# ShujiaHuang/basevar

Measured on AMD Instinct MI355X. Metric: genomic sites/sec through basetype caller at N samples, higher is better.
Workload: dtype f64

## Files before the change

basevar_amd/_capi.py:

```python
import ctypes as C
import os

import numpy as np

HERE = os.path.dirname(os.path.abspath(__file__))
LIB_PATH = os.environ.get("BASEVAR_AMD_LIB") or os.path.join(HERE, "lib", "libbasevar_amd.so")

BV_MAX_ALT = 4
BV_MAX_GROUPS = 255
BV_NO_GROUP = 0xFF
BV_MEM_DEVICE, BV_MEM_HOST = 0, 1
BV_SLAB_RPR_TAGGED, BV_RPR_TAG_MAX_RANK = 0x1, 0x1FFF
BV_FLAG_LANES = 0x10000000
BV_FLAG_SPARSE_TIMING = 0x20000000
BV_FORM_SHORT_ROWS, BV_FORM_ONE_KERNEL, BV_FORM_PASS2_FUSED = 0x1, 0x2, 0x4
BV_FLAG_TALLY_ONLY, BV_FLAG_SKIP_FISHER, BV_FLAG_SKIP_LRT, BV_FLAG_TILE_STATE, BV_FLAG_WAVE_SOLVER = 0x1, 0x2, 0x4, 0x8, 0x10
BV_OK, BV_ERR_INVALID_ARG, BV_ERR_NO_DEVICE, BV_ERR_HIP, BV_ERR_TOO_LARGE, BV_ERR_SITE = 0, -1, -2, -3, -4, -5

BV_SITE_COVERED, BV_SITE_VARIANT, BV_SITE_BAD_QUAL = 0x1, 0x2, 0x4
BV_SITE_ZERO_FREQ, BV_SITE_RANKSUM, BV_SITE_SOR_OVERFLOW, BV_SITE_RPR_RANGE = 0x8, 0x10, 0x20, 0x40

BV_CELL_REV, BV_CELL_NOCALL, BV_CELL_N, BV_CELL_INS, BV_CELL_DEL = 0x04, 0x08, 0x08, 0x09, 0x0A

SITE_DTYPE = np.dtype([
    ("depth", "<u4", 4), ("total_depth", "<u4"), ("status", "<u4"),
    ("cvg_sb", "<u4", 4), ("cvg_fs", "<f8"), ("cvg_sor", "<f8"),
    ("n_alt", "u1"), ("alt", "u1", 4), ("n_em", "u1"), ("em_iters", "<u2"),
    ("af", "<f8", 4), ("caf", "<f8", 4), ("qual", "<f8"), ("chi2", "<f8"), ("qd", "<f8"),
    ("var_sb", "<u4", 4), ("var_fs", "<f8"), ("var_sor", "<f8"),
    ("mq_ranksum", "<f8"), ("rpr_ranksum", "<f8"), ("bq_ranksum", "<f8"),
])
GROUP_DTYPE = np.dtype([("n_alt", "u1"), ("alt", "u1", 4), ("reserved", "u1", 3), ("total_depth", "<u4"),
                        ("reserved2", "<u4"), ("af", "<f8", 4)])
assert SITE_DTYPE.itemsize == 208 and GROUP_DTYPE.itemsize == 48


class Slab(C.Structure):
    _fields_ = [("n_sites", C.c_uint32), ("n_samples", C.c_uint32), ("pitch", C.c_uint64),
                ("base_strand", C.c_void_p), ("qual", C.c_void_p), ("mapq", C.c_void_p), ("rpr", C.c_void_p),
                ("ref_base", C.c_void_p), ("group_id", C.c_void_p), ("n_groups", C.c_uint32),
                ("mem_kind", C.c_uint32), ("layout", C.c_uint32), ("reserved_", C.c_uint32)]


class SparseTile(C.Structure):
    _fields_ = [("n_sites", C.c_uint32), ("n_samples", C.c_uint32), ("n_entries", C.c_uint32), ("n_groups", C.c_uint32),
                ("row_start", C.c_void_p), ("sample", C.c_void_p), ("base_strand", C.c_void_p), ("qual", C.c_void_p), ("mapq", C.c_void_p),
                ("rpr", C.c_void_p), ("group_id", C.c_void_p), ("mem_kind", C.c_uint32), ("layout", C.c_uint32)]


class TextRows(C.Structure):
    _fields_ = [("text", C.c_void_p), ("row_off", C.c_void_p), ("file_samples", C.c_void_p), ("text_bytes", C.c_uint64),
                ("n_positions", C.c_uint32), ("n_files", C.c_uint32), ("reserved_", C.c_uint32)]


BV_TEXT_SKIP, BV_TEXT_HOST, BV_TEXT_INDEL = 1, 2, 4


class BgzfMembers(C.Structure):
    _fields_ = [("data", C.c_void_p), ("member_off", C.c_void_p), ("data_bytes", C.c_uint64), ("n_members", C.c_uint32),
                ("reserved_", C.c_uint32)]


class BgzfRows(C.Structure):
    _fields_ = [("data", C.c_void_p), ("member_off", C.c_void_p), ("data_bytes", C.c_uint64), ("file_member", C.c_void_p),
                ("file_samples", C.c_void_p), ("skip_bytes", C.c_void_p), ("skip_lines", C.c_void_p), ("n_files", C.c_uint32),
                ("max_positions", C.c_uint32), ("at_end", C.c_uint32), ("reserved_", C.c_uint32)]

# ... 128 lines not shown
```

basevar_amd/csrc/bv_engine.hip:

```cpp
#include <hip/hip_runtime.h>
#include <link.h>
#include <sched.h>

#include <algorithm>
#include <cctype>
#include <cmath>
#include <cstdio>
#include <cstdlib>
#include <cstring>
#include <mutex>
#include <string>
#include <vector>

#include "bv_engine_impl.h"

void bv_launch_synth(const bv_synth_params &p, uint32_t n_sites, uint32_t n_samples, uint64_t pitch, uint8_t *bs,
                     uint8_t *q, uint8_t *mapq, uint16_t *rpr, uint8_t *ref_base, hipStream_t stream);

namespace {
std::mutex g_err_mu;
std::string g_err;

void set_global_error(const std::string &m) {
    std::lock_guard<std::mutex> lk(g_err_mu);
// ... 351 lines not shown
            e->err = std::string(#call) + ": " + hipGetErrorString(_s);                               \
            return bail(BV_ERR_HIP);                                                                  \
        }                                                                                             \
    } while (0)
    BV_TRY(hipSetDevice(cfg->device));
    e->n_cu = prop.multiProcessorCount > 0 ? (uint32_t)prop.multiProcessorCount : 256u;
    BV_TRY(hipStreamCreateWithFlags(&e->stream, hipStreamNonBlocking));
    BV_TRY(hipEventCreateWithFlags(&e->ev_done, hipEventDisableTiming));
    for (auto &tri : e->ring)
        for (auto &ev : tri) BV_TRY(hipEventCreate(&ev));
    BV_TRY(hipMalloc(&e->d_tables, sizeof(BvTables)));
    BV_TRY(hipMalloc(&e->d_var_list, sizeof(uint32_t) * (size_t)cfg->max_sites));
    BV_TRY(hipMalloc(&e->d_counters, sizeof(uint32_t) * BV_CTR_WORDS * bv_engine::kCtrBlocks));
    BV_TRY(hipHostMalloc(&e->h_counters, sizeof(uint32_t) * BV_CTR_WORDS * bv_engine::kCtrBlocks));
    std::memset(e->h_counters, 0, sizeof(uint32_t) * BV_CTR_WORDS * bv_engine::kCtrBlocks);
    BV_TRY(hipMemset(e->d_counters, 0, sizeof(uint32_t) * BV_CTR_WORDS * bv_engine::kCtrBlocks));

    BvTables t;
    const double MLN10TO10 = -0.23025850929940458;
    for (int qv = 0; qv < BV_QBINS; ++qv) {
        double epsilon = exp((double)qv * MLN10TO10);
        t.hit[qv] = 1.0 - epsilon;
        t.miss[qv] = epsilon / 3;
        t.loghit[qv] = log(t.hit[qv]);
        t.logmiss[qv] = log(t.miss[qv]);
    }
    e->host_log_exact = load_host_log_table(t.hostlog) ? 1 : 0;
    if (!e->host_log_exact) {
        static const char *note =
            "basevar_amd: note: the host libm's log() could not be reproduced on the device (no glibc __log_data table found, or it "
            "failed verification); sites of <= 64 covered samples use the device library's log(): values within 1e-6, exact ties "
            "between allele subsets undecided (records carry BV_SITE_LOG_APPROX)";
        static std::once_flag said;
        std::call_once(said, [] { if (!std::getenv("BASEVAR_AMD_QUIET")) std::fprintf(stderr, "%s\n", note); });
        set_global_error(note);
    }
    {
        size_t nfact = (size_t)(cfg->max_samples ? cfg->max_samples : 1u << 20) + 2;
        if (nfact < (1u << 16)) nfact = 1u << 16;
        if (nfact > (1u << 23)) nfact = 1u << 23;
        std::vector<double> lf(nfact);
        for (size_t k = 0; k < nfact; ++k) {
            int sign;
            lf[k] = lgamma_r((double)k + 1.0, &sign);
        }
        BV_TRY(hipMalloc(&e->d_lnfact, sizeof(double) * nfact));
        BV_TRY(hipMemcpy(e->d_lnfact, lf.data(), sizeof(double) * nfact, hipMemcpyHostToDevice));
        t.lnfact = e->d_lnfact;
        t.lnfact_n = (uint32_t)nfact;
        t.pad_ = 0;
    }
    BV_TRY(hipMemcpy(e->d_tables, &t, sizeof(t), hipMemcpyHostToDevice));
#undef BV_TRY
    if (cfg->flags & BV_FLAG_LANES) {
        if (const char *nl = std::getenv("BASEVAR_AMD_LANES")) e->n_lanes = std::max(2, std::min((int)bv_engine::kMaxLanes, std::atoi(nl)));
        for (int k = 0; k < e->n_lanes; ++k) {
            bv_engine_config c = *cfg;
            c.flags &= ~BV_FLAG_LANES;
            const int rc = bv_engine_create(&c, &e->lane[k]);
            if (rc != BV_OK) {
                const std::string m = bv_last_error(nullptr);
                bv_engine_destroy(e);
                set_global_error("bv_engine_create: lane engine: " + m);
                return rc;
            }
            e->lane[k]->is_lane = true;
        }
    }
    *out = e;
    return BV_OK;
}

int bv_engine_destroy(bv_engine *e) {
    if (!e) return BV_OK;
    (void)hipSetDevice(e->cfg.device);
    for (bv_engine *&l : e->lane) {
        if (l) (void)bv_engine_destroy(l);
        l = nullptr;
    }
    if (e->ev_entry) (void)hipEventDestroy(e->ev_entry);
    if (e->stream) (void)hipStreamSynchronize(e->stream);
    bv_text_state_free(e->text);
    bv_bgzf_state_free(e->bgzf);
    bv_deflate_state_free(e->deflate);
    for (hipStream_t st : e->used_streams) (void)hipStreamSynchronize(st);
    for (auto &tri : e->ring)
        for (auto &ev : tri)
            if (ev) (void)hipEventDestroy(ev);
    if (e->d_tables) (void)hipFree(e->d_tables);
    if (e->d_lnfact) (void)hipFree(e->d_lnfact);
    if (e->d_var_list) (void)hipFree(e->d_var_list);
    if (e->d_counters) (void)hipFree(e->d_counters);
    if (e->d_gid) (void)hipFree(e->d_gid);
    if (e->d_summ) (void)hipFree(e->d_summ);
    if (e->d_bins) (void)hipFree(e->d_bins);
    if (e->d_cand_list) (void)hipFree(e->d_cand_list);
    if (e->d_easy_list) (void)hipFree(e->d_easy_list);
    if (e->d_easy3_list) (void)hipFree(e->d_easy3_list);
    if (e->d_ovf) (void)hipFree(e->d_ovf);
    if (e->d_gitems) (void)hipFree(e->d_gitems);
    if (e->d_gidp) (void)hipFree(e->d_gidp);
    if (e->d_chain) (void)hipFree(e->d_chain);
    if (e->d_ref_cat) (void)hipFree(e->d_ref_cat);
    if (e->d_out_cat) (void)hipFree(e->d_out_cat);
    if (e->ev_done) (void)hipEventDestroy(e->ev_done);
    if (e->ev_host) (void)hipEventDestroy(e->ev_host);
    if (e->h_counters) (void)hipHostFree(e->h_counters);
    for (auto &sl : e->sring) {
        if (sl.buf) (void)hipFree(sl.buf);
        if (sl.copied) (void)hipEventDestroy(sl.copied);
        if (sl.freed) (void)hipEventDestroy(sl.freed);
    }
    tile_job_free(e->tile);
    if (e->d_gid_round) (void)hipFree(e->d_gid_round);
    if (e->d_gout_round) (void)hipFree(e->d_gout_round);
    for (hipStream_t cs : e->copy_stream)
        if (cs) (void)hipStreamSynchronize(cs);
    for (hipStream_t cs : e->copy_stream)
        if (cs) (void)hipStreamDestroy(cs);
    if (e->stream) (void)hipStreamDestroy(e->stream);
    delete e;
    return BV_OK;
}

}

int bv_impl::launch_passes(bv_engine *e, const uint8_t *bs, const uint8_t *q, const uint8_t *mq, const uint16_t *rp, const uint8_t *refb,
                           const uint8_t *gid, size_t P, uint32_t n_sites, uint32_t n_samples, uint32_t n_groups, bv_site_result *dout,
                           bv_group_result *dgout, hipStream_t st, const BvChain *chain, bool chain_cat, uint32_t layout) {
    const uint32_t rpr_tag = (layout & BV_SLAB_RPR_TAGGED) && rp != nullptr ? 1u : 0u;
    const size_t S = n_sites, G = n_groups;
    const size_t Gr = G < BV_GROUPS_PER_ROUND ? G : (size_t)BV_GROUPS_PER_ROUND, n_rounds = G ? (G + Gr - 1) / Gr : 1;
    if (n_rounds > 1 && chain != nullptr) return fail(e, BV_ERR_INVALID_ARG, "launch_passes: more than 32 pop-groups do not chain");
    if (G && chain == nullptr) BV_HIP(e, hipMemsetAsync(dgout, 0, S * G * sizeof(bv_group_result), st));
    if (n_rounds > 1) {
        int rc = grow_device(e, &e->d_gid_round, &e->d_gid_round_bytes, up256(n_samples) + 256);
        if (rc == BV_OK) rc = grow_device(e, &e->d_gout_round, &e->d_gout_round_bytes, S * Gr * sizeof(bv_group_result));
        if (rc != BV_OK) return rc;
    }

    const bool timed = !(e->cfg.flags & BV_FLAG_SPARSE_TIMING) || (e->n_launches % 8u) == 0u;
    e->n_launches += 1;
    hipEvent_t *ev = nullptr;
    if (timed) {
        if (e->ring_count == bv_engine::kRing) {
            int rc = drain_timings(e, true);
            if (rc != BV_OK) return rc;
        }
        const int slot = e->ring_head;
        e->ring_head = (e->ring_head + 1) % bv_engine::kRing;
        e->ring_count += 1;
        e->last_slot = slot;
        ev = e->ring[slot];
        e->ring_one_kernel[slot] = false;
    }
    const bool two_kernel = n_samples <= BV_SHORT_ROW_MAX;

    BvPass2Args a2;
    a2.bs = bs; a2.q = q; a2.mapq = mq; a2.rpr = rp; a2.ref_base = refb; a2.group_id = gid; a2.pitch = P;
    a2.n_sites = n_sites; a2.n_samples = n_samples; a2.n_groups = n_groups;
    a2.min_af = e->cfg.min_af; a2.tables = e->d_tables; a2.out = dout; a2.gout = dgout;
    a2.var_list = e->d_var_list; a2.counters = e->d_counters; a2.n_cu = e->n_cu; a2.flags = e->cfg.flags;
    a2.gitems = nullptr; a2.gitem_cap = 0; a2.gidp = nullptr;
    a2.ch = chain;
    a2.ch_cat = chain_cat ? 1u : 0u;
    a2.rpr_tag = rpr_tag;
    if (G && gid && dgout && !(e->cfg.flags & BV_FLAG_GROUP_INLINE)) {
        const uint64_t want64 = (uint64_t)S * Gr, most = (8192ull << 20) / (sizeof(uint32_t) * BV_P2G_ITEM_WORDS);
        uint32_t want = (uint32_t)(want64 < most ? want64 : most);
        if (want > e->gitem_cap) {
            if (e->d_gitems) BV_HIP(e, hipFree(e->d_gitems));
            e->d_gitems = nullptr; e->gitem_cap = 0;
            for (;;) {
                if (hipMalloc(&e->d_gitems, sizeof(uint32_t) * BV_P2G_ITEM_WORDS * (size_t)want) == hipSuccess) {
                    e->gitem_cap = want;
                    break;
                }
                (void)hipGetLastError();
                e->d_gitems = nullptr;
                if (want < 1024u) break;
                want /= 2u;
            }
        }
        a2.gitems = e->d_gitems; a2.gitem_cap = e->gitem_cap;
        const size_t n16 = ((size_t)n_samples + 15) & ~(size_t)15;
        const int rc = grow_device(e, &e->d_gidp, &e->d_gidp_bytes, n16 + 256);
        if (rc != BV_OK) return rc;
        a2.gidp = e->d_gidp;
        if (n_rounds == 1) {
            bv_launch_gid_prepare(gid, e->d_gidp, (uint32_t)n16, n_groups, st);
            BV_HIP(e, hipGetLastError());
        }
    }
    if (n_rounds > 1) a2.n_groups = (uint32_t)Gr;

    e->last_blocks = 1;
#ifdef BV_TEAM_DEBUG
    const bool rotate = false;
#else
    const bool rotate = true;
#endif
    uint32_t cb = 0;
    if (rotate) {
        cb = e->ctr_rot % bv_engine::kCtrBlocks;
        if (cb == 0)
            BV_HIP(e, hipMemset2DAsync(e->d_counters, sizeof(uint32_t) * BV_CTR_WORDS, 0, sizeof(uint32_t) * BV_CTR_PER_LAUNCH * BV_CTR_STRIDE,
                                       bv_engine::kCtrBlocks, st));
        e->ctr_rot += 1;
    } else {
        e->ctr_rot = 0;
        BV_HIP(e, hipMemsetAsync(e->d_counters, 0, sizeof(uint32_t) * BV_CTR_PER_LAUNCH * BV_CTR_STRIDE, st));
    }
    e->last_ctr_base = cb;
    a2.counters = e->d_counters + (size_t)cb * BV_CTR_WORDS;
    bool pass2_fused = false;
    e->last_form = two_kernel ? BV_FORM_SHORT_ROWS : 0u;
    if (ev) BV_HIP(e, hipEventRecord(ev[0], st));
    if (two_kernel) {
        if (n_sites > e->short_sites) {
            if (e->d_summ) BV_HIP(e, hipFree(e->d_summ));
            if (e->d_bins) BV_HIP(e, hipFree(e->d_bins));
            if (e->d_cand_list) BV_HIP(e, hipFree(e->d_cand_list));
            if (e->d_easy_list) BV_HIP(e, hipFree(e->d_easy_list));
            if (e->d_easy3_list) BV_HIP(e, hipFree(e->d_easy3_list));
            if (e->d_ovf) BV_HIP(e, hipFree(e->d_ovf));
            e->d_ovf = nullptr;
            e->d_summ = nullptr; e->d_bins = nullptr; e->d_cand_list = nullptr; e->d_easy_list = nullptr; e->d_easy3_list = nullptr; e->short_sites = 0;
            BV_HIP(e, hipMalloc(&e->d_summ, sizeof(BvSiteSummary) * (size_t)n_sites));
            BV_HIP(e, hipMalloc(&e->d_bins, sizeof(uint32_t) * BV_S_BIN_STRIDE * (size_t)n_sites));
            BV_HIP(e, hipMalloc(&e->d_cand_list, sizeof(uint32_t) * (size_t)n_sites));
            BV_HIP(e, hipMalloc(&e->d_easy_list, sizeof(uint32_t) * (size_t)n_sites));
            BV_HIP(e, hipMalloc(&e->d_easy3_list, sizeof(uint32_t) * (size_t)n_sites));
            BV_HIP(e, hipMalloc(&e->d_ovf, sizeof(uint32_t) * 4 * (size_t)n_sites));
            e->short_sites = n_sites;
        }
        BvP1ShortArgs s1;
        s1.bs = bs; s1.q = q; s1.ref_base = refb; s1.pitch = P; s1.n_sites = n_sites; s1.n_samples = n_samples;
        s1.flags = e->cfg.flags; s1.n_cu = e->n_cu; s1.min_af = e->cfg.min_af; s1.tables = e->d_tables; s1.out = dout;
        s1.var_list = e->d_var_list; s1.counters = e->d_counters + (size_t)cb * BV_CTR_WORDS;
        s1.summ = e->d_summ; s1.bins = e->d_bins;
        s1.cand_list = e->d_cand_list; s1.easy_list = e->d_easy_list; s1.easy3_list = e->d_easy3_list;
        s1.ovf = e->d_ovf;
        s1.ch = chain;
        s1.mapq = nullptr; s1.rpr = nullptr; s1.rpr_tag = rpr_tag;
        const uint32_t form = (e->cfg.flags >> 12) & 0xFu;
        if (form != 9u && bv_p1s_fused_takes(s1)) {
            if (ev) e->ring_one_kernel[e->last_slot] = true;
            if (form != 10u && mq != nullptr && rp != nullptr && !(e->cfg.flags & BV_FLAG_PASS2_SWEEP)) {
                s1.mapq = mq; s1.rpr = rp;
                pass2_fused = true;
            }
            bv_launch_p1s_fused(s1, st);
            BV_HIP(e, hipGetLastError());
            e->last_form |= BV_FORM_ONE_KERNEL | (pass2_fused ? BV_FORM_PASS2_FUSED : 0u);
        } else {
            bv_launch_p1s_stream(s1, st);
            BV_HIP(e, hipGetLastError());
            if (ev) BV_HIP(e, hipEventRecord(ev[3], st));
            bv_launch_p1s_solve(s1, st);
            BV_HIP(e, hipGetLastError());
        }
        if (ev) BV_HIP(e, hipEventRecord(ev[1], st));
    } else {
        if (ev) e->ring_one_kernel[e->last_slot] = true;
        BvPass1Args a1;
        a1.bs = bs; a1.q = q; a1.ref_base = refb; a1.pitch = P; a1.n_sites = n_sites;
        a1.n_samples = n_samples; a1.flags = e->cfg.flags; a1.min_af = e->cfg.min_af; a1.tables = e->d_tables; a1.out = dout;
        a1.var_list = e->d_var_list; a1.counters = e->d_counters + (size_t)cb * BV_CTR_WORDS; a1.n_cu = e->n_cu;
        a1.ch = chain;
        bv_launch_pass1(a1, st);
        BV_HIP(e, hipGetLastError());
        e->last_form |= BV_FORM_ONE_KERNEL;
        if (ev) BV_HIP(e, hipEventRecord(ev[1], st));
    }

    for (size_t r = 0; r < n_rounds; ++r) {
        const size_t g_lo = r * Gr, g_n = n_rounds > 1 ? std::min(Gr, G - g_lo) : G;
        if (n_rounds > 1) {
            const size_t n16 = ((size_t)n_samples + 15) & ~(size_t)15;
            bv_launch_gid_round(gid, e->d_gid_round, (uint32_t)n16, (uint32_t)g_lo, (uint32_t)g_n, st);
            BV_HIP(e, hipGetLastError());
            bv_launch_gid_prepare(e->d_gid_round, e->d_gidp, (uint32_t)n16, (uint32_t)g_n, st);
            BV_HIP(e, hipGetLastError());
            BV_HIP(e, hipMemsetAsync(e->d_gout_round, 0, S * g_n * sizeof(bv_group_result), st));
        }
        BvPass2Args ac = a2;
        if (n_rounds > 1) { ac.group_id = e->d_gid_round; ac.n_groups = (uint32_t)g_n; ac.gout = e->d_gout_round; }
        if (pass2_fused || r > 0) {
            if (G == 0) continue;
            ac.mapq = nullptr; ac.rpr = nullptr;
        }
        bv_launch_pass2(ac, st);
        BV_HIP(e, hipGetLastError());
        bv_launch_p2g_solve16(ac, st);
        BV_HIP(e, hipGetLastError());
        if (n_rounds > 1)
            BV_HIP(e, hipMemcpy2DAsync(dgout + g_lo, G * sizeof(bv_group_result), e->d_gout_round, g_n * sizeof(bv_group_result),
                                       g_n * sizeof(bv_group_result), S, hipMemcpyDeviceToDevice, st));
    }
    if (ev) BV_HIP(e, hipEventRecord(ev[2], st));

    if (rotate) e->ctr_mirror_stale = true;
    else BV_HIP(e, hipMemcpyAsync(e->h_counters, e->d_counters, sizeof(uint32_t) * BV_CTR_WORDS * bv_engine::kCtrBlocks, hipMemcpyDeviceToHost, st));
    const int rc = copy_records_back(e, st);
    if (rc != BV_OK) return rc;
    e->submitted = true;
    return mark_done(e, st);
}

extern "C" {

int bv_engine_submit(bv_engine *e, const bv_slab *slab, bv_site_result *out, bv_group_result *gout, void *stream_) {
    if (!e) return fail(nullptr, BV_ERR_INVALID_ARG, "bv_engine_submit: null engine");
    if (!slab || !out) return fail(e, BV_ERR_INVALID_ARG, "bv_engine_submit: null slab/out");
    if (slab->n_sites == 0) return fail(e, BV_ERR_INVALID_ARG, "bv_engine_submit: n_sites == 0");
    if (slab->n_sites > e->cfg.max_sites)
        return fail(e, BV_ERR_TOO_LARGE, "bv_engine_submit: n_sites exceeds cfg.max_sites");
    if (slab->n_samples == 0 || slab->pitch < slab->n_samples || (slab->pitch & 15ull))
        return fail(e, BV_ERR_INVALID_ARG, "bv_engine_submit: pitch must be >= n_samples and a multiple of 16");
    if (!slab->base_strand || !slab->qual || !slab->ref_base)
        return fail(e, BV_ERR_INVALID_ARG, "bv_engine_submit: base_strand, qual and ref_base planes are required");
    if ((slab->mapq == nullptr) != (slab->rpr == nullptr))
        return fail(e, BV_ERR_INVALID_ARG, "bv_engine_submit: mapq and rpr planes must be given together");
    if (slab->n_groups > BV_MAX_GROUPS)
        return fail(e, BV_ERR_INVALID_ARG, "bv_engine_submit: n_groups exceeds BV_MAX_GROUPS");
    if (slab->n_groups > 0 && (!slab->group_id || !gout))
        return fail(e, BV_ERR_INVALID_ARG, "bv_engine_submit: n_groups > 0 needs group_id and gout");
    auto misaligned = [](const void *p) { return (reinterpret_cast<uintptr_t>(p) & 15u) != 0; };
    if (misaligned(slab->base_strand) || misaligned(slab->qual) || misaligned(slab->mapq) || misaligned(slab->rpr))
// ... 7 lines not shown
    if ((e->cfg.flags & BV_FLAG_LANES) && !e->is_lane && slab->mem_kind != BV_MEM_HOST) {
        const int k = (int)(e->lane_next++ % (unsigned)e->n_lanes);
        if (!e->lane[k]) {
            bv_engine_config c = e->cfg;
            c.flags &= ~BV_FLAG_LANES;
            int rc = bv_engine_create(&c, &e->lane[k]);
            if (rc != BV_OK) return fail(e, rc, std::string("bv_engine_submit: lane engine: ") + bv_last_error(nullptr));
            e->lane[k]->is_lane = true;
        }
        bv_engine *l = e->lane[k];
        hipStream_t src = stream_ ? (hipStream_t)stream_ : e->stream;
        if (hipStreamQuery(src) != hipSuccess) {
            (void)hipGetLastError();
            if (!e->ev_entry) BV_HIP(e, hipEventCreateWithFlags(&e->ev_entry, hipEventDisableTiming));
            BV_HIP(e, hipEventRecord(e->ev_entry, src));
            BV_HIP(e, hipStreamWaitEvent(l->stream, e->ev_entry, 0));
        }
        const int rc = bv_engine_submit(l, slab, out, gout, nullptr);
        if (rc != BV_OK) return fail(e, rc, bv_last_error(l));
        e->last_lane = k;
        e->submitted = true;
        return BV_OK;
    }
    e->last_lane = -1;
    hipStream_t st = stream_ ? (hipStream_t)stream_ : e->stream;
    {
        int rc = use_stream(e, st);
        if (rc != BV_OK) return rc;
    }

    const uint8_t *bs = slab->base_strand, *q = slab->qual, *mq = slab->mapq, *refb = slab->ref_base,
                  *gid = slab->group_id;
    const uint16_t *rp = slab->rpr;
    bv_site_result *dout = out;
    bv_group_result *dgout = gout;
    const size_t S = slab->n_sites, P = slab->pitch, G = slab->n_groups;
    StageSlot *slot = nullptr;
    if (slab->mem_kind == BV_MEM_HOST) {
        HostPlane pl[5] = {{bs, S * P, nullptr}, {q, S * P, nullptr}, {mq, mq ? S * P : 0, nullptr},
                           {rp, rp ? S * P * 2 : 0, nullptr}, {refb, S, nullptr}};
        const int rc = stage_records(e, pl, 5, S, G, out, gout, &slot, &dout, &dgout, st);
        if (rc != BV_OK) return rc;
        bs = pl[0].dev; q = pl[1].dev; mq = pl[2].dev;
        rp = reinterpret_cast<const uint16_t *>(pl[3].dev);
        refb = pl[4].dev;
    } else {
        e->host_out = nullptr; e->host_gout = nullptr;
    }
    if (G) {
        int rc = stage_group_ids(e, slab->group_id, slab->n_samples, slab->mem_kind == BV_MEM_HOST, st, &gid);
        if (rc != BV_OK) return rc;
    }

    int rc = launch_passes(e, bs, q, mq, rp, refb, gid, P, slab->n_sites, slab->n_samples, slab->n_groups, dout, dgout, st, nullptr, false, slab->layout);
    if (rc == BV_OK && slot) rc = stage_release(e, slot, st);
    return rc;
}

int bv_engine_submit_many(bv_engine *e, uint32_t n_slabs, const bv_slab *slabs, bv_site_result *const *outs, void *stream_) {
    return bv_engine_submit_many_g(e, n_slabs, slabs, outs, nullptr, stream_);
}

int bv_engine_submit_many_g(bv_engine *e, uint32_t n_slabs, const bv_slab *slabs, bv_site_result *const *outs,
                            bv_group_result *const *gouts, void *stream_) {
    if (!e) return fail(nullptr, BV_ERR_INVALID_ARG, "bv_engine_submit_many: null engine");
    if (!slabs || !outs || n_slabs == 0) return fail(e, BV_ERR_INVALID_ARG, "bv_engine_submit_many: null / empty argument");
    bool chainable = n_slabs > 1;
    uint64_t total = 0;
    auto misaligned = [](const void *p) { return (reinterpret_cast<uintptr_t>(p) & 15u) != 0; };
    for (uint32_t k = 0; k < n_slabs; ++k) {
        const bv_slab &s = slabs[k];
        if (!outs[k]) return fail(e, BV_ERR_INVALID_ARG, "bv_engine_submit_many: null record buffer");
        if (s.n_sites == 0 || s.n_samples == 0 || s.pitch < s.n_samples || (s.pitch & 15ull) || !s.base_strand || !s.qual || !s.ref_base ||
            (s.mapq == nullptr) != (s.rpr == nullptr) || misaligned(s.base_strand) || misaligned(s.qual) || misaligned(s.mapq) ||
            misaligned(s.rpr) || (s.mem_kind != BV_MEM_HOST && misaligned(outs[k])) || s.n_groups > BV_MAX_GROUPS || (s.layout & ~BV_SLAB_RPR_TAGGED) || s.reserved_)
            return fail(e, BV_ERR_INVALID_ARG, "bv_engine_submit_many: a slab fails the checks of bv_engine_submit");
        if (s.n_groups > 0 && (!s.group_id || !gouts || !gouts[k]))
            return fail(e, BV_ERR_INVALID_ARG, "bv_engine_submit_many: a slab with pop-groups needs group_id and its gouts[k] (bv_engine_submit_many_g)");
        if (s.n_sites > e->cfg.max_sites) return fail(e, BV_ERR_TOO_LARGE, "bv_engine_submit_many: a slab exceeds cfg.max_sites");
        chainable = chainable && s.mem_kind != BV_MEM_HOST && !(e->cfg.flags & (BV_FLAG_PASS2_SWEEP | BV_FLAG_GROUP_INLINE)) &&
                    s.n_samples == slabs[0].n_samples && s.pitch == slabs[0].pitch && (s.mapq == nullptr) == (slabs[0].mapq == nullptr) &&
                    s.n_groups == slabs[0].n_groups && (s.n_groups == 0 || s.group_id == slabs[0].group_id) && s.layout == slabs[0].layout;
        total += s.n_sites;
    }
    const uint32_t G = slabs[0].n_groups;
    if (chainable && G && (uint64_t)std::min<uint64_t>(total, e->cfg.max_sites) * G * sizeof(uint32_t) * BV_P2G_ITEM_WORDS > (8192ull << 20)) chainable = false;
    if (G > BV_GROUPS_PER_ROUND) chainable = false;
    if (!chainable) {
        for (uint32_t k = 0; k < n_slabs; ++k) {
            int rc = bv_engine_submit(e, &slabs[k], outs[k], slabs[k].n_groups ? gouts[k] : nullptr, stream_);
            if (rc != BV_OK) return rc;
        }
        return BV_OK;
    }
    if (total > e->cfg.max_sites) return fail(e, BV_ERR_TOO_LARGE, "bv_engine_submit_many: the slabs together exceed cfg.max_sites");
    BV_HIP(e, hipSetDevice(e->cfg.device));
    hipStream_t st = stream_ ? (hipStream_t)stream_ : e->stream;
    {
        int rc = use_stream(e, st);
        if (rc != BV_OK) return rc;
    }
    e->host_out = nullptr; e->host_gout = nullptr;
    e->last_lane = -1;
    const size_t P = slabs[0].pitch;
    const bool ranks = slabs[0].mapq != nullptr;
    const uint8_t *gid = nullptr;
    if (G) {
// ... 442 lines not shown
```

basevar_amd/csrc/bv_engine_impl.h:

```cpp
#pragma once

#include <hip/hip_runtime.h>

#include <mutex>
#include <string>
#include <vector>

#include "bv_kernels.h"

struct BvTextState;
void bv_text_state_free(BvTextState *t);
struct BvBgzfState;
void bv_bgzf_state_free(BvBgzfState *t);
struct BvDeflateState;
void bv_deflate_state_free(BvDeflateState *t);

struct bv_engine {
    bv_engine_config cfg;
    hipStream_t stream = nullptr;
    hipStream_t last_stream = nullptr;
    std::vector<hipStream_t> used_streams;
    hipEvent_t ev_host = nullptr;
    hipEvent_t ev_done = nullptr;
    bool ev_done_set = false;
// ... 35 lines not shown
    BvChain *d_chain = nullptr;
    uint8_t *d_ref_cat = nullptr;
    bv_site_result *d_out_cat = nullptr;
    unsigned chain_next = 0;
    uint32_t acc_n = 0;
    bool submitted = false;
    static constexpr int kStage = 4;
    struct StageSlot {
        void *buf = nullptr;
        size_t bytes = 0;
        hipEvent_t copied = nullptr, freed = nullptr;
        hipStream_t cs = nullptr;
        bool used = false;
    };
    StageSlot sring[kStage];
    unsigned sring_next = 0;
    hipStream_t copy_stream[2] = {nullptr, nullptr};
    bv_site_result *stage_out = nullptr;
    bv_group_result *stage_gout = nullptr;
    bv_site_result *host_out = nullptr;
    bv_group_result *host_gout = nullptr;
    size_t host_out_bytes = 0, host_gout_bytes = 0;
    struct TileJob {
        struct Job {
            bool open = false;
            bool join = false;
            bool ranks = false;
            uint32_t sites = 0, groups = 0, samples_total = 0, samples_seen = 0;
            uint32_t layout = 0;
            bool layout_set = false;
            bool filled = false;
            size_t pitch = 0, o_q = 0, o_mq = 0, o_rp = 0, o_gid = 0;
            uint32_t stride = 0, rank_win = 1024, hg_off = 0, ord_off = 0;
        } job;
        uint8_t *rows = nullptr;
        size_t rows_bytes = 0;
        uint32_t *state = nullptr, *maxr = nullptr;
        size_t state_bytes = 0, maxr_bytes = 0;
        uint32_t *ovf = nullptr;
        static constexpr uint32_t kOvfCap = 1u << 22;
        static constexpr int kDescRing = 4;
        void *h_desc[kDescRing] = {}, *d_desc[kDescRing] = {};
        hipEvent_t ev_desc[kDescRing] = {};
        bool desc_used[kDescRing] = {};
        unsigned desc_next = 0;
    } tile;
    static constexpr int kMaxLanes = 4;
    bv_engine *lane[kMaxLanes] = {nullptr, nullptr, nullptr, nullptr};
    int n_lanes = 2;
    unsigned lane_next = 0;
    int last_lane = -1;
    bool is_lane = false;
    hipEvent_t ev_entry = nullptr;
    BvTextState *text = nullptr;
    BvBgzfState *bgzf = nullptr;
    BvDeflateState *deflate = nullptr;
    mutable std::mutex mu;
    std::string err;
};

namespace bv_impl {
using StageSlot = bv_engine::StageSlot;

int fail(bv_engine *e, int code, const std::string &msg);
#define BV_HIP(e, call)                                                                                  \
    do {                                                                                                 \
        hipError_t _s = (call);                                                                          \
        if (_s != hipSuccess)                                                                            \
            return ::bv_impl::fail((e), BV_ERR_HIP, std::string(#call) + ": " + hipGetErrorString(_s));  \
    } while (0)

inline size_t up256(size_t x) { return (x + 255) & ~(size_t)255; }

template <class S>
S *engine_state(bv_engine *e, S *&state) {
    if (!state) {
        state = new S();
        state->device = e->cfg.device;
    }
    return state;
}

template <class T>
int grow_device(bv_engine *e, T **buf, size_t *bytes, size_t need) {
    if (need <= *bytes) return BV_OK;
    if (*buf) BV_HIP(e, hipFree(*buf));
    *buf = nullptr; *bytes = 0;
    BV_HIP(e, hipMalloc(buf, need));
    *bytes = need;
    return BV_OK;
}

int use_stream(bv_engine *e, hipStream_t st);
int mark_done(bv_engine *e, hipStream_t st);

int stage_acquire(bv_engine *e, size_t bytes, StageSlot **out);
int stage_order(bv_engine *e, StageSlot *sl, hipStream_t st);
int stage_publish(bv_engine *e, StageSlot *sl, hipStream_t st);
int stage_release(bv_engine *e, StageSlot *sl, hipStream_t st);
struct HostPlane {
    const void *src;
    size_t bytes;
    const uint8_t *dev;
};
struct HostPlanes {
    const uint8_t *lo = nullptr, *hi = nullptr;
    bool one_copy = false;
    size_t bytes = 0;
};
HostPlanes plan_host_planes(const HostPlane *pl, int n);
int copy_host_planes(bv_engine *e, HostPlane *pl, int n, const HostPlanes &h, uint8_t *base, hipStream_t cs);
int stage_host_planes(bv_engine *e, HostPlane *pl, int n, size_t extra, StageSlot **slot_out, uint8_t **extra_dev, hipStream_t st);
int stage_records(bv_engine *e, HostPlane *pl, int n, size_t S, size_t G, bv_site_result *out, bv_group_result *gout, StageSlot **slot,
                  bv_site_result **dout, bv_group_result **dgout, hipStream_t st);
int copy_records_back(bv_engine *e, hipStream_t st);

int stage_group_ids(bv_engine *e, const uint8_t *gid, uint32_t n_samples, bool host, hipStream_t st, const uint8_t **out);
int launch_passes(bv_engine *e, const uint8_t *bs, const uint8_t *q, const uint8_t *mq, const uint16_t *rp, const uint8_t *refb,
                  const uint8_t *gid, size_t P, uint32_t n_sites, uint32_t n_samples, uint32_t n_groups, bv_site_result *dout,
                  bv_group_result *dgout, hipStream_t st, const BvChain *chain = nullptr ,
                  bool chain_cat = false , uint32_t layout = 0 );
void tile_job_free(bv_engine::TileJob &t);
}
```

basevar_amd/csrc/bv_kernels.h:

```cpp
#pragma once

#include "bv_device.h"

#define BV_CTR_STRIDE 32u
#define BV_CTR_VARIANTS (0u * BV_CTR_STRIDE)
#define BV_CTR_TICKET (1u * BV_CTR_STRIDE)
#define BV_CTR_CANDS (2u * BV_CTR_STRIDE)
#define BV_CTR_EASY (3u * BV_CTR_STRIDE)
#define BV_CTR_EASY3 (4u * BV_CTR_STRIDE)
#define BV_TICKET_SLICES 8u
#define BV_CTR_TICKET_A (5u * BV_CTR_STRIDE)
#define BV_CTR_TICKET_B ((5u + BV_TICKET_SLICES) * BV_CTR_STRIDE)
#define BV_CTR_PER_LAUNCH (5u + 2u * BV_TICKET_SLICES)
#define BV_CTR_ZEROFREQ (BV_CTR_PER_LAUNCH * BV_CTR_STRIDE)
#define BV_CTR_TIMEOUT ((BV_CTR_PER_LAUNCH + 1u) * BV_CTR_STRIDE)
#define BV_CTR_WORDS ((BV_CTR_PER_LAUNCH + 2u) * BV_CTR_STRIDE)
#define BV_TMO_PUSH 0x1u
#define BV_TMO_PUSH_VARIANT 0x100u
#define BV_TMO_TAKE 0x10000u
#define BV_TMO_TAKE_VARIANT 0x1000000u
#define BV_TMO_RING 0x10000000u

#define BV_MAX_CHAIN 16
struct BvChain {
    uint32_t n;
    uint32_t first[BV_MAX_CHAIN];
    const uint8_t *bs[BV_MAX_CHAIN], *q[BV_MAX_CHAIN], *mapq[BV_MAX_CHAIN], *ref_base[BV_MAX_CHAIN];
    const uint16_t *rpr[BV_MAX_CHAIN];
    bv_site_result *out[BV_MAX_CHAIN];
    bv_group_result *gout[BV_MAX_CHAIN];
};
#if defined(__HIPCC__)
typedef const __attribute__((address_space(4))) BvChain *BvChainC;
__device__ __forceinline__ BvChainC bv_chain_const(const BvChain *p) { return (BvChainC)(uintptr_t)p; }
__device__ __forceinline__ uint32_t bv_chain_seg(BvChainC c, uint32_t site) {
    uint32_t k = 0;
    const uint32_t n = c->n;
#pragma unroll
    for (int i = 1; i < BV_MAX_CHAIN; ++i) k += ((uint32_t)i < n && site >= c->first[i]) ? 1u : 0u;
    return k;
}
#endif

struct BvPass1Args {
    const uint8_t *bs;
    const uint8_t *q;
    const uint8_t *ref_base;
    uint64_t pitch;
    uint32_t n_sites;
    uint32_t n_samples;
    uint32_t flags;
    double min_af;
    const BvTables *tables;
    bv_site_result *out;
    uint32_t *var_list;
    uint32_t *counters;
    uint32_t n_cu;
    const BvChain *ch;
};

struct BvPass2Args {
    const uint8_t *bs;
    const uint8_t *q;
    const uint8_t *mapq;
    const uint16_t *rpr;
    const uint8_t *ref_base;
    const uint8_t *group_id;
    uint64_t pitch;
    uint32_t n_sites;
    uint32_t n_samples;
    uint32_t n_groups;
    double min_af;
    const BvTables *tables;
    bv_site_result *out;
    bv_group_result *gout;
    const uint32_t *var_list;
    const uint32_t *counters;
    uint32_t n_cu;
    uint32_t flags;
    uint32_t *gitems;
    uint32_t gitem_cap;
    const uint8_t *gidp;
    const BvChain *ch;
    uint32_t ch_cat;
    uint32_t rpr_tag;
};
#define BV_P2G_ITEM_WORDS (8u + BV_SLOTS * BV_WAVE)
#define BV_G16_SLOTS 8
#define BV_G16_MAX_BINS (16 * BV_G16_SLOTS)
#define BV_G16_GRP_WORDS 288
#define BV_P2G_PENDING 0x80000000u
#define BV_P2G_HARD 0x40000000u
#define BV_P2G_SHALLOW 0x20000000u
#define BV_P2G_L4 0x10000000u
#define BV_P2G_L8 0x08000000u

#define BV_SHORT_ROW_MAX 49152u
#define BV_S_BIN_STRIDE 512u
struct __attribute__((aligned(16))) BvSiteSummary {
    uint32_t fwd[4], rev[4];
    uint32_t nb;
    uint32_t flags;
    uint32_t pad_[2];
};
#define BV_SUM_Q0_MASK 0xFu
#define BV_SUM_BADQ 0x10u
#define BV_SUM_CAND 0x20u
struct BvP1ShortArgs {
    const uint8_t *bs, *q, *ref_base;
    uint64_t pitch;
    uint32_t n_sites, n_samples, flags, n_cu;
// ... 136 lines not shown
```

basevar_amd/csrc/bv_pass1.hip:

```cpp
#include "bv_kernels.h"

#include "bv_solver.h"
#include "bv_tally.h"

#define BV_RING_EXTRA 2
template <int NBUF, int NSOLVE>
struct __attribute__((aligned(16))) BvPass1Shared {
    uint32_t hist[NBUF][BV_H2_WORDS];
    uint32_t published[NBUF];
    uint32_t filled[NBUF];
    uint32_t drained[NBUF];
    uint32_t site_of[NBUF];
    uint32_t swz_of[NBUF];
    uint32_t dense_hint;
    double tab_hit[BV_QBINS], tab_miss[BV_QBINS];
    BvSolverShared sv[NSOLVE];
};

#define BV_TALLY_U 4
struct BvChunkSet {
    bv_u32x4 vb[BV_TALLY_U], vq[BV_TALLY_U];
};
template <bool FULL>
__device__ __forceinline__ void bv_chunks_load(BvChunkSet &c, const uint8_t *bs_row, const uint8_t *q_row, uint32_t base,
// ... 404 lines not shown
                    if (hist[b << 8] + hist[(b | 4) << 8]) S.q0_mask |= 1u << b;
                bv_prologue_wave<false>(hist, bin_code, bin_cnt, lane, S.fwd, S.rev, &S.nb, &S.badq);
                bv_lrt_sync<0>();
                BvHqFromHist hq{hist};
                bool team = bv_team_takes(sa.flags, S);
                if (team) {
                    team = __hip_atomic_load(&tm->helpers, __ATOMIC_ACQUIRE, __HIP_MEMORY_SCOPE_WORKGROUP) == (uint32_t)NTALLY;
                    if (!team && tm->last_site == site) {
                        bv_wait_flag(&tm->helpers, (uint32_t)NTALLY, &a.counters[BV_CTR_TIMEOUT]);
                        team = true;
                    }
                }
#ifdef BV_TEAM_DEBUG
                const unsigned long long t0_ = __builtin_readcyclecounter();
#endif
                if (team) {
                    ++jobs;
                    if (lane == 0) { tm->site = site; tm->buf = buf; tm->lrt.bar = 0u; }
                    bv_set_flag(&tm->gen, jobs);
                    BvTeamWork<NTALLY> work;
                    work.tm = tm; work.job = jobs; work.err = &a.counters[BV_CTR_TIMEOUT];
                    bv_site_solve<false, BvHqFromHist, false, BvTeamWork<NTALLY>>(sa, site, S, bin_code, bin_cnt, hq, sv, sh.tab_hit,
                                                                                 sh.tab_miss, lane, work);
                    bv_wait_flag(&tm->done, jobs * (uint32_t)NTALLY, &a.counters[BV_CTR_TIMEOUT]);
                } else {
                    bv_site_solve<false>(sa, site, S, bin_code, bin_cnt, hq, sv, sh.tab_hit, sh.tab_miss, lane);
                }
#ifdef BV_TEAM_DEBUG
                if (lane == 0) {
                    const uint32_t dt = (uint32_t)((__builtin_readcyclecounter() - t0_) >> 6);
                    atomicAdd(&a.counters[team ? BV_CTR_CANDS : BV_CTR_EASY3], 1u);
                    atomicAdd(&a.counters[(team ? BV_CTR_CANDS : BV_CTR_EASY3) + 1], dt);
                }
#endif
            } else {
                bv_solve_site_wave<false>(sa, site, (BV_LDS uint32_t *)sh.hist[buf], (BV_LDS uint32_t *)sh.sv[s].bin_code,
                                          (BV_LDS uint32_t *)sh.sv[s].bin_cnt, (BV_LDS BvSolverScratch *)&sh.sv[s].sc,
                                          (BV_LDS const double *)sh.tab_hit, (BV_LDS const double *)sh.tab_miss, lane);
            }
            if (lane == 0) sh.dense_hint = (sh.sv[s].sc.res.total_depth >= (a.n_samples >> 2)) ? 1u : 0u;
            uint4 *h4 = reinterpret_cast<uint4 *>(sh.hist[buf]);
#pragma unroll
            for (int i = 0; i < BV_H2_WORDS / 4 / BV_WAVE; ++i) h4[i * BV_WAVE + lane] = make_uint4(0, 0, 0, 0);
            bv_set_flag(&sh.drained[buf], gen + 1u);
        }
    }
}

template <int NTALLY, int MODE>
static void bv_launch_pass1_cfg(const BvPass1Args &a, hipStream_t stream) {
    constexpr int NSOLVE = 1;
    constexpr uint32_t by_vgpr = 16u / (NTALLY + NSOLVE);
    constexpr uint32_t by_lds = (uint32_t)((160u * 1024u) / sizeof(BvPass1Shared<NSOLVE + BV_RING_EXTRA, NSOLVE>));
    uint32_t grid = (a.n_cu ? a.n_cu : 256u) * (by_vgpr < by_lds ? by_vgpr : by_lds);
    if (grid > a.n_sites) grid = a.n_sites;
    const dim3 block(64 * (NTALLY + NSOLVE));
    if (a.ch != nullptr) hipLaunchKernelGGL((bv_pass1_kernel<NTALLY, NSOLVE, true, MODE>), dim3(grid), block, 0, stream, a);
    else hipLaunchKernelGGL((bv_pass1_kernel<NTALLY, NSOLVE, false, MODE>), dim3(grid), block, 0, stream, a);
}

void bv_launch_pass1(const BvPass1Args &a, hipStream_t stream) {
    if (a.n_sites <= (uint32_t)BV_TEAM_MAX_SITES && ((a.flags >> 8) & 0xFu) != 2u) bv_launch_pass1_cfg<3, 1>(a, stream);
    else bv_launch_pass1_cfg<3, 2>(a, stream);
}
```

include/basevar_amd_diag.h:

```cpp
#ifndef BASEVAR_AMD_DIAG_H
#define BASEVAR_AMD_DIAG_H

#include "basevar_amd.h"

#ifdef __cplusplus
extern "C" {
#endif

#define BV_FLAG_TALLY_ONLY 0x1u
#define BV_FLAG_SKIP_FISHER 0x2u
#define BV_FLAG_SKIP_LRT 0x4u
#define BV_FLAG_GRID_LIMIT(n) (((uint32_t)(n) & 0xFFu) << 16)
#define BV_FLAG_GROUP_INLINE 0x40u
#define BV_FLAG_PASS2_SWEEP 0x20u
#define BV_FLAG_NO_DOM 0x1000000u
#define BV_FLAG_P2_TAIL_DMA 0x2000000u
#define BV_FLAG_WAVE_SOLVER 0x10u
#define BV_FLAG_LONG_ROW_FORM(n) (((uint32_t)(n) & 0xFu) << 8)
#define BV_FLAG_SHORT_ROW_FORM(n) (((uint32_t)(n) & 0xFu) << 12)
#define BV_FLAG_FAULT_LOST_HANDOFF 0x40000000u

#define BV_FORM_SHORT_ROWS 0x1u
#define BV_FORM_ONE_KERNEL 0x2u
#define BV_FORM_PASS2_FUSED 0x4u
int bv_engine_last_launch_form(bv_engine *e, uint32_t *form);

int bv_engine_kernel_ms(bv_engine *e, float *pass1_ms, float *pass2_ms);

int bv_engine_timing_reset(bv_engine *e);
int bv_engine_timing_get(bv_engine *e, double *pass1_total_ms, double *pass2_total_ms, uint32_t *n_submits);
int bv_engine_timing_get_ex(bv_engine *e, double *stream_total_ms, double *pass1_total_ms, double *pass2_total_ms,
                            uint32_t *n_submits);

#define BV_HOST_LOG_TABLE_DOUBLES 274
int bv_host_log_probe(double *table);
double bv_host_log_eval(const double *table, double x);
int bv_engine_host_log_eval(bv_engine *e, const double *x, double *y, uint32_t n);

typedef struct bv_synth_params {
    uint64_t seed;
    uint64_t site_offset;
    float coverage;
    float indel_frac;
    float qual_mean, qual_sd;
    uint32_t qual_min, qual_max;
    uint32_t layout;
    uint32_t reserved_;
} bv_synth_params;

int bv_synth_fill(int device, const bv_synth_params *p, uint32_t n_sites, uint32_t n_samples,
                  uint64_t pitch, uint8_t *base_strand, uint8_t *qual, uint8_t *mapq,
                  uint16_t *rpr, uint8_t *ref_base, void *stream);

#ifdef __cplusplus
}
#endif
#endif
```

Measured before the change: 22.72 million.

## Split single-kernel slab across two streams to overlap pass1/pass2 partitions

For mid-sized slabs without groups or chaining, the sites are split roughly 45/55 and each part runs its pass1 and pass2 on a separate stream, with separate counter blocks and fork/join events. The first part's pass1 grid is capped at two workgroups per CU so the second stream can occupy the remaining CUs, and the form choice uses the full site count. The goal is to let one part's pass2 overlap the other part's pass1 and to fill idle CUs during tail phases. The cost is extra launches and event synchronization, plus possible contention between the two partitions.

```diff
diff --git a/basevar_amd/_capi.py b/basevar_amd/_capi.py
--- a/basevar_amd/_capi.py
+++ b/basevar_amd/_capi.py
@@ -13,6 +13,7 @@
 BV_SLAB_RPR_TAGGED, BV_RPR_TAG_MAX_RANK = 0x1, 0x1FFF
 BV_FLAG_LANES = 0x10000000
 BV_FLAG_SPARSE_TIMING = 0x20000000
+BV_FLAG_NO_SPLIT = 0x4000000
 BV_FORM_SHORT_ROWS, BV_FORM_ONE_KERNEL, BV_FORM_PASS2_FUSED = 0x1, 0x2, 0x4
 BV_FLAG_TALLY_ONLY, BV_FLAG_SKIP_FISHER, BV_FLAG_SKIP_LRT, BV_FLAG_TILE_STATE, BV_FLAG_WAVE_SOLVER = 0x1, 0x2, 0x4, 0x8, 0x10
 BV_OK, BV_ERR_INVALID_ARG, BV_ERR_NO_DEVICE, BV_ERR_HIP, BV_ERR_TOO_LARGE, BV_ERR_SITE = 0, -1, -2, -3, -4, -5
diff --git a/basevar_amd/csrc/bv_engine.hip b/basevar_amd/csrc/bv_engine.hip
--- a/basevar_amd/csrc/bv_engine.hip
+++ b/basevar_amd/csrc/bv_engine.hip
@@ -427,6 +427,7 @@
     }
     BV_TRY(hipMemcpy(e->d_tables, &t, sizeof(t), hipMemcpyHostToDevice));
 #undef BV_TRY
+    if (const char *ms = std::getenv("BASEVAR_AMD_SPLIT_MIN_SITES")) e->split_min_sites = (uint32_t)std::max(2l, std::atol(ms));
     if (cfg->flags & BV_FLAG_LANES) {
         if (const char *nl = std::getenv("BASEVAR_AMD_LANES")) e->n_lanes = std::max(2, std::min((int)bv_engine::kMaxLanes, std::atoi(nl)));
         for (int k = 0; k < e->n_lanes; ++k) {
@@ -455,6 +456,7 @@
     }
     if (e->ev_entry) (void)hipEventDestroy(e->ev_entry);
     if (e->stream) (void)hipStreamSynchronize(e->stream);
+    if (e->split_stream) (void)hipStreamSynchronize(e->split_stream);
     bv_text_state_free(e->text);
     bv_bgzf_state_free(e->bgzf);
     bv_deflate_state_free(e->deflate);
@@ -493,6 +495,9 @@
         if (cs) (void)hipStreamSynchronize(cs);
     for (hipStream_t cs : e->copy_stream)
         if (cs) (void)hipStreamDestroy(cs);
+    if (e->split_stream) (void)hipStreamDestroy(e->split_stream);
+    if (e->ev_fork) (void)hipEventDestroy(e->ev_fork);
+    if (e->ev_join) (void)hipEventDestroy(e->ev_join);
     if (e->stream) (void)hipStreamDestroy(e->stream);
     delete e;
     return BV_OK;
@@ -500,9 +505,22 @@
 
 }
 
+#ifndef BV_SPLIT_A_PERCENT
+#define BV_SPLIT_A_PERCENT 45u
+#endif
+#ifndef BV_SPLIT_MAX_SITES
+#define BV_SPLIT_MAX_SITES 65536u
+#endif
+#ifndef BV_SPLIT_WG_A
+#define BV_SPLIT_WG_A 2u
+#endif
+#ifndef BV_SPLIT_WG_B
+#define BV_SPLIT_WG_B 0u
+#endif
+
 int bv_impl::launch_passes(bv_engine *e, const uint8_t *bs, const uint8_t *q, const uint8_t *mq, const uint16_t *rp, const uint8_t *refb,
                            const uint8_t *gid, size_t P, uint32_t n_sites, uint32_t n_samples, uint32_t n_groups, bv_site_result *dout,
-                           bv_group_result *dgout, hipStream_t st, const BvChain *chain, bool chain_cat, uint32_t layout) {
+                           bv_group_result *dgout, hipStream_t st, const BvChain *chain, bool chain_cat, uint32_t layout, bool may_split) {
     const uint32_t rpr_tag = (layout & BV_SLAB_RPR_TAGGED) && rp != nullptr ? 1u : 0u;
     const size_t S = n_sites, G = n_groups;
     const size_t Gr = G < BV_GROUPS_PER_ROUND ? G : (size_t)BV_GROUPS_PER_ROUND, n_rounds = G ? (G + Gr - 1) / Gr : 1;
@@ -575,13 +593,36 @@
 #else
     const bool rotate = true;
 #endif
+    bool split = may_split && rotate && !two_kernel && G == 0 && chain == nullptr && !e->is_lane && !(e->cfg.flags & BV_FLAG_NO_SPLIT) &&
+                 n_sites >= 2u && n_sites >= e->split_min_sites && n_sites <= BV_SPLIT_MAX_SITES;
+    if (split) {
+        hipStreamCaptureStatus cap = hipStreamCaptureStatusNone;
+        if (hipStreamIsCapturing(st, &cap) != hipSuccess) {
+            (void)hipGetLastError();
+            split = false;
+        } else if (cap != hipStreamCaptureStatusNone) {
+            split = false;
+        }
+    }
+    bool st_busy = true;
+    if (split) {
+        if (!e->split_stream) {
+            BV_HIP(e, hipStreamCreateWithFlags(&e->split_stream, hipStreamNonBlocking));
+            BV_HIP(e, hipEventCreateWithFlags(&e->ev_fork, hipEventDisableTiming));
+            BV_HIP(e, hipEventCreateWithFlags(&e->ev_join, hipEventDisableTiming));
+        }
+        st_busy = hipStreamQuery(st) != hipSuccess;
+        (void)hipGetLastError();
+        if (e->ctr_rot % bv_engine::kCtrBlocks == bv_engine::kCtrBlocks - 1u) e->ctr_rot += 1;
+    }
     uint32_t cb = 0;
     if (rotate) {
         cb = e->ctr_rot % bv_engine::kCtrBlocks;
         if (cb == 0)
             BV_HIP(e, hipMemset2DAsync(e->d_counters, sizeof(uint32_t) * BV_CTR_WORDS, 0, sizeof(uint32_t) * BV_CTR_PER_LAUNCH * BV_CTR_STRIDE,
                                        bv_engine::kCtrBlocks, st));
-        e->ctr_rot += 1;
+        e->ctr_rot += split ? 2u : 1u;
+        if (split) e->last_blocks = 2;
     } else {
         e->ctr_rot = 0;
         BV_HIP(e, hipMemsetAsync(e->d_counters, 0, sizeof(uint32_t) * BV_CTR_PER_LAUNCH * BV_CTR_STRIDE, st));
@@ -636,6 +677,46 @@
             BV_HIP(e, hipGetLastError());
         }
         if (ev) BV_HIP(e, hipEventRecord(ev[1], st));
+    } else if (split) {
+        if (ev) e->ring_one_kernel[e->last_slot] = true;
+        hipStream_t s2 = e->split_stream;
+        uint32_t nA = (uint32_t)((uint64_t)n_sites * BV_SPLIT_A_PERCENT / 100u);
+        if (nA == 0u) nA = 1u;
+        const size_t off = (size_t)nA * P;
+        if (st_busy || cb == 0u) {
+            BV_HIP(e, hipEventRecord(e->ev_fork, st));
+            BV_HIP(e, hipStreamWaitEvent(s2, e->ev_fork, 0));
+        }
+        BvPass1Args a1;
+        a1.bs = bs; a1.q = q; a1.ref_base = refb; a1.pitch = P; a1.n_sites = nA;
+        a1.n_samples = n_samples; a1.flags = e->cfg.flags; a1.min_af = e->cfg.min_af; a1.tables = e->d_tables; a1.out = dout;
+        a1.var_list = e->d_var_list; a1.counters = e->d_counters + (size_t)cb * BV_CTR_WORDS; a1.n_cu = e->n_cu;
+        a1.ch = nullptr;
+        a1.wg_per_cu = BV_SPLIT_WG_A;
+#ifndef BV_SPLIT_FORM_BY_PART
+        a1.form_sites = n_sites;
+#endif
+        BvPass1Args b1 = a1;
+        b1.bs = bs + off; b1.q = q + off; b1.ref_base = refb + nA; b1.out = dout + nA; b1.n_sites = n_sites - nA;
+        b1.var_list = e->d_var_list + nA; b1.counters = a1.counters + BV_CTR_WORDS;
+        b1.wg_per_cu = BV_SPLIT_WG_B;
+        bv_launch_pass1(a1, st);
+        BV_HIP(e, hipGetLastError());
+        bv_launch_pass1(b1, s2);
+        BV_HIP(e, hipGetLastError());
+        e->last_form |= BV_FORM_ONE_KERNEL;
+        if (ev) BV_HIP(e, hipEventRecord(ev[1], s2));
+        BvPass2Args pa = a2, pb = a2;
+        pa.n_sites = nA;
+        pb.bs = bs + off; pb.q = q + off; pb.mapq = mq ? mq + off : nullptr; pb.rpr = rp ? rp + off : nullptr;
+        pb.ref_base = refb + nA; pb.out = dout + nA; pb.n_sites = n_sites - nA;
+        pb.var_list = e->d_var_list + nA; pb.counters = a2.counters + BV_CTR_WORDS;
+        bv_launch_pass2(pa, st);
+        BV_HIP(e, hipGetLastError());
+        bv_launch_pass2(pb, s2);
+        BV_HIP(e, hipGetLastError());
+        BV_HIP(e, hipEventRecord(e->ev_join, s2));
+        BV_HIP(e, hipStreamWaitEvent(st, e->ev_join, 0));
     } else {
         if (ev) e->ring_one_kernel[e->last_slot] = true;
         BvPass1Args a1;
@@ -649,7 +730,7 @@
         if (ev) BV_HIP(e, hipEventRecord(ev[1], st));
     }
 
-    for (size_t r = 0; r < n_rounds; ++r) {
+    for (size_t r = 0; r < n_rounds && !split; ++r) {
         const size_t g_lo = r * Gr, g_n = n_rounds > 1 ? std::min(Gr, G - g_lo) : G;
         if (n_rounds > 1) {
             const size_t n16 = ((size_t)n_samples + 15) & ~(size_t)15;
@@ -763,7 +844,7 @@
         if (rc != BV_OK) return rc;
     }
 
-    int rc = launch_passes(e, bs, q, mq, rp, refb, gid, P, slab->n_sites, slab->n_samples, slab->n_groups, dout, dgout, st, nullptr, false, slab->layout);
+    int rc = launch_passes(e, bs, q, mq, rp, refb, gid, P, slab->n_sites, slab->n_samples, slab->n_groups, dout, dgout, st, nullptr, false, slab->layout, true);
     if (rc == BV_OK && slot) rc = stage_release(e, slot, st);
     return rc;
 }
diff --git a/basevar_amd/csrc/bv_engine_impl.h b/basevar_amd/csrc/bv_engine_impl.h
--- a/basevar_amd/csrc/bv_engine_impl.h
+++ b/basevar_amd/csrc/bv_engine_impl.h
@@ -111,6 +111,9 @@
     int last_lane = -1;
     bool is_lane = false;
     hipEvent_t ev_entry = nullptr;
+    hipStream_t split_stream = nullptr;
+    hipEvent_t ev_fork = nullptr, ev_join = nullptr;
+    uint32_t split_min_sites = 4096;
     BvTextState *text = nullptr;
     BvBgzfState *bgzf = nullptr;
     BvDeflateState *deflate = nullptr;
@@ -178,6 +181,7 @@
 int launch_passes(bv_engine *e, const uint8_t *bs, const uint8_t *q, const uint8_t *mq, const uint16_t *rp, const uint8_t *refb,
                   const uint8_t *gid, size_t P, uint32_t n_sites, uint32_t n_samples, uint32_t n_groups, bv_site_result *dout,
                   bv_group_result *dgout, hipStream_t st, const BvChain *chain = nullptr ,
-                  bool chain_cat = false , uint32_t layout = 0 );
+                  bool chain_cat = false , uint32_t layout = 0 ,
+                  bool may_split = false );
 void tile_job_free(bv_engine::TileJob &t);
 }
diff --git a/basevar_amd/csrc/bv_kernels.h b/basevar_amd/csrc/bv_kernels.h
--- a/basevar_amd/csrc/bv_kernels.h
+++ b/basevar_amd/csrc/bv_kernels.h
@@ -57,6 +57,8 @@
     uint32_t *counters;
     uint32_t n_cu;
     const BvChain *ch;
+    uint32_t wg_per_cu = 0;
+    uint32_t form_sites = 0;
 };
 
 struct BvPass2Args {
diff --git a/basevar_amd/csrc/bv_pass1.hip b/basevar_amd/csrc/bv_pass1.hip
--- a/basevar_amd/csrc/bv_pass1.hip
+++ b/basevar_amd/csrc/bv_pass1.hip
@@ -480,7 +480,9 @@
     constexpr int NSOLVE = 1;
     constexpr uint32_t by_vgpr = 16u / (NTALLY + NSOLVE);
     constexpr uint32_t by_lds = (uint32_t)((160u * 1024u) / sizeof(BvPass1Shared<NSOLVE + BV_RING_EXTRA, NSOLVE>));
-    uint32_t grid = (a.n_cu ? a.n_cu : 256u) * (by_vgpr < by_lds ? by_vgpr : by_lds);
+    uint32_t per_cu = by_vgpr < by_lds ? by_vgpr : by_lds;
+    if (a.wg_per_cu && a.wg_per_cu < per_cu) per_cu = a.wg_per_cu;
+    uint32_t grid = (a.n_cu ? a.n_cu : 256u) * per_cu;
     if (grid > a.n_sites) grid = a.n_sites;
     const dim3 block(64 * (NTALLY + NSOLVE));
     if (a.ch != nullptr) hipLaunchKernelGGL((bv_pass1_kernel<NTALLY, NSOLVE, true, MODE>), dim3(grid), block, 0, stream, a);
@@ -488,6 +490,7 @@
 }
 
 void bv_launch_pass1(const BvPass1Args &a, hipStream_t stream) {
-    if (a.n_sites <= (uint32_t)BV_TEAM_MAX_SITES && ((a.flags >> 8) & 0xFu) != 2u) bv_launch_pass1_cfg<3, 1>(a, stream);
+    const uint32_t form_sites = a.form_sites ? a.form_sites : a.n_sites;
+    if (form_sites <= (uint32_t)BV_TEAM_MAX_SITES && ((a.flags >> 8) & 0xFu) != 2u) bv_launch_pass1_cfg<3, 1>(a, stream);
     else bv_launch_pass1_cfg<3, 2>(a, stream);
 }
diff --git a/include/basevar_amd_diag.h b/include/basevar_amd_diag.h
--- a/include/basevar_amd_diag.h
+++ b/include/basevar_amd_diag.h
@@ -15,6 +15,7 @@
 #define BV_FLAG_PASS2_SWEEP 0x20u
 #define BV_FLAG_NO_DOM 0x1000000u
 #define BV_FLAG_P2_TAIL_DMA 0x2000000u
+#define BV_FLAG_NO_SPLIT 0x4000000u
 #define BV_FLAG_WAVE_SOLVER 0x10u
 #define BV_FLAG_LONG_ROW_FORM(n) (((uint32_t)(n) & 0xFu) << 8)
 #define BV_FLAG_SHORT_ROW_FORM(n) (((uint32_t)(n) & 0xFu) << 12)
```

After: 22.29 million. 0.981x the previous value.
